# GATECH-EIC/PipeGCN

Hardware: AMD Instinct MI355X
Metric: epoch time (s), reddit 3-layer GraphSAGE (full-graph, pipelined) (lower is better)
Workload: dtype fp32; 1 GPU; model=graphsage-3L-h256, graph=reddit, num_nodes=232965, avg_degree=492, n_feat=602, n_class=41, pipeline=True, use_pp=False, norm=layer, parallelism=graph-partition dp1, num_halo=0, num_edges=114851422

## Files before the change

pipegcn_amd/csrc/bindings.cpp:

```cpp

#include "common.h"

static torch::Tensor spmm(torch::Tensor indptr, torch::Tensor indices,
                          torch::Tensor feat, torch::Tensor dst_scale,
                          torch::Tensor src_scale, torch::Tensor row_order,
                          int64_t num_rows) {
  if (feat.is_cuda()) {
    auto out = torch::empty({num_rows, feat.size(1)}, feat.options());
    spmm_csr_hip(indptr, indices, feat, dst_scale, src_scale, row_order,
                 out);
    return out;
  }
  if (feat.scalar_type() == torch::kBFloat16) {
    return spmm_cpu(indptr, indices, feat.to(torch::kFloat), dst_scale,
                    src_scale, num_rows)
        .to(torch::kBFloat16);
  }
  return spmm_cpu(indptr, indices, feat, dst_scale, src_scale, num_rows);
}

static torch::Tensor pack_rows(torch::Tensor x) {
  TORCH_CHECK(x.is_cuda() && x.dim() == 2, "pack_rows is the GPU path");
  auto packed = torch::empty({x.size(0), packed_layout(x.size(1)).stride_words},
                             x.options().dtype(torch::kInt));
  pack_rows_hip(x, packed);
  return packed;
}

static torch::Tensor spmm_packed(torch::Tensor indptr, torch::Tensor indices,
                                 torch::Tensor packed, int64_t F,
                                 torch::Tensor dst_scale,
                                 torch::Tensor row_order, int64_t num_rows) {
  TORCH_CHECK(packed.is_cuda(), "spmm_packed is the GPU path");
  auto out = torch::empty({num_rows, F},
                          packed.options().dtype(torch::kFloat));
  spmm_packed_hip(indptr, indices, packed, F, dst_scale, row_order, out);
  return out;
}

static torch::Tensor gather_rows(torch::Tensor src, torch::Tensor idx) {
  if (src.is_cuda()) {
    auto out = torch::empty({idx.numel(), src.size(1)}, src.options());
    gather_rows_hip(src, idx, out);
    return out;
  }
  return src.index_select(0, idx);
}

static void gather_rows_out(torch::Tensor src, torch::Tensor idx,
                            torch::Tensor out) {
  if (src.is_cuda()) {
    gather_rows_hip(src, idx, out);
  } else {
    torch::index_select_out(out, src, 0, idx);
  }
}

static void scatter_add_rows(torch::Tensor dst, torch::Tensor idx,
                             torch::Tensor src) {
  if (dst.is_cuda()) {
    scatter_add_rows_hip(dst, idx, src);
  } else {
    dst.index_add_(0, idx, src);
  }
}

static torch::Tensor sage_dual_gemm(torch::Tensor x1, torch::Tensor x2,
                                    torch::Tensor w1, torch::Tensor w2,
                                    torch::Tensor bias) {
  if (x1.is_cuda()) {
    auto out = torch::empty({x1.size(0), w1.size(0)}, x1.options());
// ... 23 lines not shown
  auto mask = torch::empty({(x.numel() + 7) / 8},
                           x.options().dtype(torch::kUInt8));
  dropout_fwd_hip(x, y, mask, p, seed);
  return {y, mask};
}

static torch::Tensor dropout_bwd(torch::Tensor dy, torch::Tensor mask,
                                 double p) {
  auto dx = torch::empty_like(dy);
  dropout_bwd_hip(dy.contiguous(), mask, dx, p);
  return dx;
}

static std::vector<torch::Tensor> layer_norm_relu_fwd(torch::Tensor x,
                                                      torch::Tensor w,
                                                      torch::Tensor b,
                                                      double eps, bool relu) {
  TORCH_CHECK(x.is_cuda(), "fused layer_norm_relu is the GPU path");
  auto y = torch::empty_like(x);
  auto xhat = torch::empty_like(x);
  auto rstd = torch::empty({x.size(0)}, x.options().dtype(torch::kFloat));
  layer_norm_relu_fwd_hip(x.contiguous(), w, b, eps, relu, y, xhat, rstd);
  return {y, xhat, rstd};
}

static std::vector<torch::Tensor> layer_norm_relu_bwd(
    torch::Tensor dy, torch::Tensor xhat, torch::Tensor rstd,
    torch::Tensor w, torch::Tensor b, bool relu) {
  auto dx = torch::empty_like(dy);
  const int64_t N = dy.size(0);
  const int64_t F = dy.size(1);
  const int64_t nblk = std::min<int64_t>(1024, (N + 3) / 4);
  auto dw_part = torch::empty({nblk * 4, F},
                              dy.options().dtype(torch::kFloat));
  auto db_part = torch::empty_like(dw_part);
  layer_norm_relu_bwd_hip(dy.contiguous(), xhat, rstd, w, b, relu, dx,
                          dw_part, db_part);
  return {dx, colsum_hip(dw_part), colsum_hip(db_part)};
}

static void ema_update(torch::Tensor avg, torch::Tensor x, double momentum) {
  if (avg.is_cuda()) {
    ema_update_hip(avg, x, momentum);
  } else {
    avg.mul_(momentum).add_(x, 1.0 - momentum);
  }
}

PYBIND11_MODULE(TORCH_EXTENSION_NAME, m) {
  m.doc() = "pipegcn_amd native core (gfx950 HIP kernels + host graph ops)";
  m.def("build_csr", &build_csr, "COO -> CSR (counting sort by dst)");
  m.def("partition_graph", &partition_graph_cpu,
        "BFS-grown + refined k-way partitioner (cut/vol objective)");
  m.def("spmm", &spmm, "CSR SpMM with fused scale epilogue (fwd & transpose)");
  m.def("pack_rows", &pack_rows,
        "fp32 [N, F] -> packed rows int32 [N, stride_words]");
  m.def("spmm_packed", &spmm_packed,
        "CSR SpMM over packed rows (fp32, dst_scale epilogue)");
  m.def("gather_rows", &gather_rows, "out[i,:] = src[idx[i],:]");
  m.def("gather_rows_out", &gather_rows_out,
        "gather into a preallocated out buffer");
  m.def("scatter_add_rows", &scatter_add_rows, "dst[idx[i],:] += src[i,:]");
  m.def("ema_update", &ema_update, "avg = m*avg + (1-m)*x");
  m.def("colsum", &colsum, "out[n] = sum_m x[m,n]");
  m.def("sage_dual_gemm", &sage_dual_gemm,
        "out = x1 @ w1^T + x2 @ w2^T + bias (MFMA fp32, fused)");
  m.def("dual_dgrad", &dual_dgrad_hip,
        "gx1 = g w1, gx2 = g w2 fused MFMA dgrad");
  m.def("dual_wgrad", &dual_wgrad_hip,
        "gw1 = g^T x1 [, gw2 = g^T x2] fused MFMA split-M wgrad");
  m.def("dropout_fwd", &dropout_fwd,
        "fused dropout, bitpacked mask -> (y, mask)");
  m.def("dropout_bwd", &dropout_bwd, "dx = mask ? dy/(1-p) : 0");
  m.def("layer_norm_relu_fwd", &layer_norm_relu_fwd,
        "fused LayerNorm[+ReLU] -> (y, xhat, rstd)");
  m.def("layer_norm_relu_bwd", &layer_norm_relu_bwd,
        "-> (dx, dweight, dbias)");
  m.def("gat_row_stats", &gat_row_stats_hip,
        "per-destination log-sum-exp of the GAT edge scores -> lse");
  m.def("gat_aggregate_fwd", &gat_aggregate_fwd_hip,
        "edge-softmax aggregation -> (out[, zc, csum])", py::arg("indptr"),
        py::arg("indices"), py::arg("z"), py::arg("el"), py::arg("er"),
        py::arg("lse"), py::arg("row_order"), py::arg("num_cols"),
        py::arg("num_heads"), py::arg("slope"), py::arg("with_aux"),
        py::arg("drop_key") = 0, py::arg("drop_thr") = 0,
        py::arg("drop_scale") = 1.0);
  m.def("gat_aggregate_bwd", &gat_aggregate_bwd_hip,
        "transpose edge-softmax aggregation over the CSC -> (dz, d_el)",
        py::arg("indptr"), py::arg("indices"), py::arg("g"), py::arg("z"),
        py::arg("el"), py::arg("er"), py::arg("lse"), py::arg("t"),
        py::arg("row_order"), py::arg("num_cols"), py::arg("num_heads"),
        py::arg("slope"), py::arg("drop_key") = 0, py::arg("drop_thr") = 0,
        py::arg("drop_scale") = 1.0);
  m.def("gat_dropout_keep", &gat_dropout_keep_hip,
        "attention-dropout keep bits of explicit (u, v) ids -> bool [n, H]",
        py::arg("u"), py::arg("v"), py::arg("num_heads"), py::arg("seed"),
        py::arg("p"));
  m.def("gatv2_fwd", &gatv2_fwd_hip,
        "GATv2 dynamic-attention aggregation over the CSR -> (out, lse)",
        py::arg("indptr"), py::arg("indices"), py::arg("zl"), py::arg("zr"),
        py::arg("attn"), py::arg("row_order"), py::arg("num_cols"),
        py::arg("num_heads"), py::arg("slope"), py::arg("drop_key") = 0,
        py::arg("drop_thr") = 0, py::arg("drop_scale") = 1.0);
  m.def("gatv2_bwd_dst", &gatv2_bwd_dst_hip,
        "GATv2 backward over the CSR -> (d_zr, pa)", py::arg("indptr"),
        py::arg("indices"), py::arg("g"), py::arg("zl"), py::arg("zr"),
        py::arg("attn"), py::arg("lse"), py::arg("t"), py::arg("row_order"),
// ... 13 lines not shown
```

pipegcn_amd/csrc/common.h:

```cpp
#pragma once

#include <torch/extension.h>

#include <cstdint>
#include <vector>


std::vector<torch::Tensor> build_csr(torch::Tensor u, torch::Tensor v,
                                     int64_t num_rows);

torch::Tensor partition_graph_cpu(torch::Tensor indptr, torch::Tensor indices,
                                  int64_t nparts, int64_t objective,
                                  double balance_slack, int64_t n_refine_passes,
                                  int64_t seed);

torch::Tensor spmm_cpu(torch::Tensor indptr, torch::Tensor indices,
                       torch::Tensor feat, torch::Tensor dst_scale,
                       torch::Tensor src_scale, int64_t num_rows);


void spmm_csr_hip(torch::Tensor indptr, torch::Tensor indices,
                  torch::Tensor feat, torch::Tensor dst_scale,
                  torch::Tensor src_scale, torch::Tensor row_order,
                  torch::Tensor out);

struct PackedLayout {
  int64_t mask_words;
  int64_t hdr_words;
  int64_t stride_words;
};
PackedLayout packed_layout(int64_t F);
void pack_rows_hip(torch::Tensor x, torch::Tensor packed);
void spmm_packed_hip(torch::Tensor indptr, torch::Tensor indices,
                     torch::Tensor packed, int64_t F, torch::Tensor dst_scale,
                     torch::Tensor row_order, torch::Tensor out);

void gather_rows_hip(torch::Tensor src, torch::Tensor idx, torch::Tensor out);

void scatter_add_rows_hip(torch::Tensor dst, torch::Tensor idx,
                          torch::Tensor src);

void ema_update_hip(torch::Tensor avg, torch::Tensor x, double momentum);

torch::Tensor colsum_hip(torch::Tensor x);

void dropout_fwd_hip(torch::Tensor x, torch::Tensor y, torch::Tensor mask,
                     double p, int64_t seed);
void dropout_bwd_hip(torch::Tensor dy, torch::Tensor mask, torch::Tensor dx,
                     double p);

void layer_norm_relu_fwd_hip(torch::Tensor x, torch::Tensor w,
                             torch::Tensor b, double eps, bool relu,
                             torch::Tensor y, torch::Tensor xhat,
                             torch::Tensor rstd);
std::vector<torch::Tensor> dual_dgrad_hip(torch::Tensor g, torch::Tensor w1,
                                          torch::Tensor w2);

std::vector<torch::Tensor> dual_wgrad_hip(torch::Tensor g, torch::Tensor x1,
                                          torch::Tensor x2);

void layer_norm_relu_bwd_hip(torch::Tensor dy, torch::Tensor xhat,
                             torch::Tensor rstd, torch::Tensor w,
                             torch::Tensor b, bool relu, torch::Tensor dx,
                             torch::Tensor dw_part, torch::Tensor db_part);

torch::Tensor gat_row_stats_hip(torch::Tensor indptr, torch::Tensor indices,
                                torch::Tensor el, torch::Tensor er,
                                int64_t num_cols, double slope);
std::vector<torch::Tensor> gat_aggregate_fwd_hip(
    torch::Tensor indptr, torch::Tensor indices, torch::Tensor z,
    torch::Tensor el, torch::Tensor er, torch::Tensor lse,
    torch::Tensor row_order, int64_t num_cols, int64_t H, double slope,
    bool with_aux, int64_t drop_key, int64_t drop_thr, double drop_scale);
std::vector<torch::Tensor> gat_aggregate_bwd_hip(
    torch::Tensor indptr, torch::Tensor indices, torch::Tensor g,
    torch::Tensor z, torch::Tensor el, torch::Tensor er, torch::Tensor lse,
    torch::Tensor t, torch::Tensor row_order, int64_t num_cols, int64_t H,
// ... 24 lines not shown
```

pipegcn_amd/csrc/hip/elementwise.hip:

```cpp

#include "../common.h"
#include "hip_util.h"

#include <hip/hip_bf16.h>
#include <hip/hip_runtime.h>

namespace {

__device__ inline void from_f32(float v, float* p) { *p = v; }
__device__ inline void from_f32(float v, __hip_bfloat16* p) {
  *p = __float2bfloat16(v);
}

__device__ inline float wave_sum(float v) {
#pragma unroll
  for (int off = 32; off > 0; off >>= 1) v += __shfl_xor(v, off, 64);
  return v;
}

__device__ inline uint64_t splitmix64(uint64_t z) {
  z += 0x9E3779B97F4A7C15ull;
  z = (z ^ (z >> 30)) * 0xBF58476D1CE4E5B9ull;
  z = (z ^ (z >> 27)) * 0x94D049BB133111EBull;
  return z ^ (z >> 31);
// ... 206 lines not shown
    float h[LN_MAXCH][LN_VEC];
    float s1 = 0.f, s2 = 0.f;
#pragma unroll
    for (int c = 0; c < LN_MAXCH; ++c) {
      if (c >= nch) break;
#pragma unroll
      for (int k = 0; k < LN_VEC; ++k) {
        const int f = (c * 64 + lane) * LN_VEC + k;
        float gg = 0.f, hh = 0.f;
        if (f < F) {
          hh = to_f32(hr[f]);
          gg = to_f32(dyr[f]);
          if (RELU && w[f] * hh + b[f] <= 0.f) gg = 0.f;
          acc_db[c][k] += gg;
          acc_dw[c][k] += gg * hh;
          gg *= w[f];
        }
        g[c][k] = gg;
        h[c][k] = hh;
        s1 += gg;
        s2 += gg * hh;
      }
    }
    s1 = wave_sum(s1) / F;
    s2 = wave_sum(s2) / F;
    T* dxr = dx + row * F;
#pragma unroll
    for (int c = 0; c < LN_MAXCH; ++c) {
      if (c >= nch) break;
#pragma unroll
      for (int k = 0; k < LN_VEC; ++k) {
        const int f = (c * 64 + lane) * LN_VEC + k;
        if (f >= F) break;
        from_f32(rs * (g[c][k] - s1 - h[c][k] * s2), &dxr[f]);
      }
    }
  }

  float* dwp = dw_part + wid * F;
  float* dbp = db_part + wid * F;
#pragma unroll
  for (int c = 0; c < LN_MAXCH; ++c) {
    if (c >= nch) break;
#pragma unroll
    for (int k = 0; k < LN_VEC; ++k) {
      const int f = (c * 64 + lane) * LN_VEC + k;
      if (f >= F) break;
      dwp[f] = acc_dw[c][k];
      dbp[f] = acc_db[c][k];
    }
  }
}

}

void dropout_fwd_hip(torch::Tensor x, torch::Tensor y, torch::Tensor mask,
                     double p, int64_t seed) {
  TORCH_CHECK(x.is_cuda() && x.is_contiguous() && y.is_contiguous());
  TORCH_CHECK(mask.scalar_type() == torch::kUInt8 && mask.is_contiguous());
  const int64_t n = x.numel();
  TORCH_CHECK(mask.numel() >= (n + 7) / 8);
  TORCH_CHECK(p >= 0.0 && p < 1.0);
  const uint32_t p16 = static_cast<uint32_t>(p * 65536.0 + 0.5);
  const float scale = 1.f / (1.f - p16 / 65536.f);
  const int64_t groups = (n + 7) / 8;
  const int threads = 256;
  const int64_t blocks =
      std::min<int64_t>((groups + threads - 1) / threads, 65535 * 8);
  const bool bf16 = x.scalar_type() == torch::kBFloat16;
  TORCH_CHECK(bf16 || x.scalar_type() == torch::kFloat);
  if (bf16)
    hipLaunchKernelGGL(HIP_KERNEL_NAME(dropout_fwd_kernel<__hip_bfloat16>),
                       dim3(blocks), dim3(threads), 0, current_stream(),
                       reinterpret_cast<__hip_bfloat16*>(x.data_ptr()),
                       reinterpret_cast<__hip_bfloat16*>(y.data_ptr()),
                       mask.data_ptr<uint8_t>(), (uint64_t)seed, p16, scale,
                       n);
  else
    hipLaunchKernelGGL(HIP_KERNEL_NAME(dropout_fwd_kernel<float>),
                       dim3(blocks), dim3(threads), 0, current_stream(),
                       x.data_ptr<float>(), y.data_ptr<float>(),
                       mask.data_ptr<uint8_t>(), (uint64_t)seed, p16, scale,
                       n);
  check_launch();
}

void dropout_bwd_hip(torch::Tensor dy, torch::Tensor mask, torch::Tensor dx,
                     double p) {
  TORCH_CHECK(dy.is_cuda() && dy.is_contiguous() && dx.is_contiguous());
  const int64_t n = dy.numel();
  const uint32_t p16 = static_cast<uint32_t>(p * 65536.0 + 0.5);
  const float scale = 1.f / (1.f - p16 / 65536.f);
  const int64_t groups = (n + 7) / 8;
  const int threads = 256;
  const int64_t blocks =
      std::min<int64_t>((groups + threads - 1) / threads, 65535 * 8);
  const bool bf16 = dy.scalar_type() == torch::kBFloat16;
  if (bf16)
    hipLaunchKernelGGL(HIP_KERNEL_NAME(dropout_bwd_kernel<__hip_bfloat16>),
                       dim3(blocks), dim3(threads), 0, current_stream(),
                       reinterpret_cast<__hip_bfloat16*>(dy.data_ptr()),
                       mask.data_ptr<uint8_t>(),
                       reinterpret_cast<__hip_bfloat16*>(dx.data_ptr()),
                       scale, n);
  else
    hipLaunchKernelGGL(HIP_KERNEL_NAME(dropout_bwd_kernel<float>),
// ... 80 lines not shown
```

pipegcn_amd/csrc/hip/kernels.hip:

```cpp

#include "../common.h"
#include "hip_util.h"

#include <hip/hip_bf16.h>
#include <hip/hip_runtime.h>

#include <cstdlib>
#include <vector>

namespace {

__device__ __forceinline__ void st_nt(float* p, float v) {
  __builtin_nontemporal_store(v, p);
}
__device__ __forceinline__ void st_nt(__hip_bfloat16* p, float v) {
  union {
    __hip_bfloat16 b;
    unsigned short u;
  } cv;
  cv.b = __float2bfloat16(v);
  __builtin_nontemporal_store(cv.u, reinterpret_cast<unsigned short*>(p));
}
__device__ __forceinline__ void st(float* p, float v) { *p = v; }
__device__ __forceinline__ void st(__hip_bfloat16* p, float v) {
  *p = __float2bfloat16(v);
}


template <typename T, int VEC, bool HAS_SRC_SCALE>
__global__ void spmm_csr_kernel(const int64_t* __restrict__ indptr,
                                const int32_t* __restrict__ indices,
                                const T* __restrict__ feat,
                                const float* __restrict__ dst_scale,
                                const float* __restrict__ src_scale,
                                const int32_t* __restrict__ row_order,
                                T* __restrict__ out, int64_t num_rows,
                                int64_t F, int64_t nchunks) {
  const int wave_in_block =
      __builtin_amdgcn_readfirstlane(static_cast<int>(threadIdx.x) / kWave);
  const int64_t waves_per_block = blockDim.x / kWave;
  const int64_t wave_global =
      static_cast<int64_t>(blockIdx.x) * waves_per_block + wave_in_block;
  const int lane = threadIdx.x & (kWave - 1);
  const int64_t nwaves = static_cast<int64_t>(gridDim.x) * waves_per_block;
  const int64_t npairs = num_rows * nchunks;

  for (int64_t pair = wave_global; pair < npairs; pair += nwaves) {
    int64_t r = pair / nchunks;
    const int64_t chunk = pair % nchunks;
    if (row_order) r = row_order[r];
    const int64_t f0 = chunk * (kWave * VEC) + lane * VEC;
    if (f0 >= F) continue;
    const bool full = (f0 + VEC <= F);

    float acc[VEC];
#pragma unroll
    for (int k = 0; k < VEC; ++k) acc[k] = 0.f;

    const int64_t e_begin = indptr[r];
    const int64_t e_end = indptr[r + 1];
    int64_t e = e_begin;

    if (full) {
      for (; e < e_end && (e & 3); ++e) {
        const int64_t u = indices[e];
        const float s = HAS_SRC_SCALE ? src_scale[u] : 1.f;
#pragma unroll
        for (int k = 0; k < VEC; ++k)
          acc[k] += s * to_f32(feat[u * F + f0 + k]);
      }
      for (; e + 4 <= e_end; e += 4) {
        const int32x4 uu = *reinterpret_cast<const int32x4*>(indices + e);
        const int64_t u0 = uu[0];
        const int64_t u1 = uu[1];
        const int64_t u2 = uu[2];
        const int64_t u3 = uu[3];
        float s0 = 1.f, s1 = 1.f, s2 = 1.f, s3 = 1.f;
        if (HAS_SRC_SCALE) {
          s0 = src_scale[u0];
          s1 = src_scale[u1];
          s2 = src_scale[u2];
          s3 = src_scale[u3];
        }
        float v0[VEC], v1[VEC], v2[VEC], v3[VEC];
#pragma unroll
        for (int k = 0; k < VEC; ++k) v0[k] = to_f32(feat[u0 * F + f0 + k]);
#pragma unroll
        for (int k = 0; k < VEC; ++k) v1[k] = to_f32(feat[u1 * F + f0 + k]);
#pragma unroll
        for (int k = 0; k < VEC; ++k) v2[k] = to_f32(feat[u2 * F + f0 + k]);
#pragma unroll
        for (int k = 0; k < VEC; ++k) v3[k] = to_f32(feat[u3 * F + f0 + k]);
        if (HAS_SRC_SCALE) {
#pragma unroll
          for (int k = 0; k < VEC; ++k)
            acc[k] += s0 * v0[k] + s1 * v1[k] + s2 * v2[k] + s3 * v3[k];
        } else {
#pragma unroll
          for (int k = 0; k < VEC; ++k)
            acc[k] += v0[k] + v1[k] + v2[k] + v3[k];
        }
      }
      for (; e < e_end; ++e) {
        const int64_t u = indices[e];
        const float s = HAS_SRC_SCALE ? src_scale[u] : 1.f;
#pragma unroll
        for (int k = 0; k < VEC; ++k)
          acc[k] += s * to_f32(feat[u * F + f0 + k]);
      }
      const float s = dst_scale ? dst_scale[r] : 1.f;
#pragma unroll
      for (int k = 0; k < VEC; ++k) st_nt(out + r * F + f0 + k, acc[k] * s);
    } else {
      for (; e < e_end; ++e) {
        const int64_t u = indices[e];
        const float s = HAS_SRC_SCALE ? src_scale[u] : 1.f;
        for (int k = 0; k < VEC && f0 + k < F; ++k)
          acc[k] += s * to_f32(feat[u * F + f0 + k]);
      }
      const float s = dst_scale ? dst_scale[r] : 1.f;
      for (int k = 0; k < VEC && f0 + k < F; ++k)
        st(out + r * F + f0 + k, acc[k] * s);
    }
  }
}

template <typename T, int VEC>
void launch_spmm(const int64_t* indptr, const int32_t* indices,
                 const T* feat, const float* dst_scale,
                 const float* src_scale, const int32_t* row_order, T* out,
                 int64_t num_rows, int64_t F, hipStream_t stream) {
  const int64_t nchunks = (F + kWave * VEC - 1) / (kWave * VEC);
  constexpr int threads = 256;
  static_assert(threads % kWave == 0);
  const int64_t blocks = grid_for(num_rows * nchunks, threads);
  auto launch = [&](auto kern) {
    hipLaunchKernelGGL(kern, dim3(blocks), dim3(threads), 0, stream, indptr,
                       indices, feat, dst_scale, src_scale, row_order, out,
                       num_rows, F, nchunks);
  };
  if (src_scale)
    launch(HIP_KERNEL_NAME(spmm_csr_kernel<T, VEC, true>));
  else
    launch(HIP_KERNEL_NAME(spmm_csr_kernel<T, VEC, false>));
  check_launch();
}


template <typename T, int VEC, bool SCATTER_ADD>
__global__ void rowcopy_kernel(const T* __restrict__ src,
                               const int64_t* __restrict__ idx,
                               T* __restrict__ dst, int64_t nrows,
                               int64_t F, int64_t nchunks) {
  const int64_t wave_global =
      (static_cast<int64_t>(blockIdx.x) * blockDim.x + threadIdx.x) / kWave;
  const int lane = threadIdx.x & (kWave - 1);
  const int64_t nwaves =
      (static_cast<int64_t>(gridDim.x) * blockDim.x) / kWave;
  const int64_t npairs = nrows * nchunks;
  for (int64_t pair = wave_global; pair < npairs; pair += nwaves) {
    const int64_t i = pair / nchunks;
    const int64_t f0 = pair % nchunks * (kWave * VEC) + lane * VEC;
    if (f0 >= F) continue;
    const int64_t j = idx[i];
    if (f0 + VEC <= F) {
#pragma unroll
      for (int k = 0; k < VEC; ++k) {
        if (SCATTER_ADD)
          st(dst + j * F + f0 + k, to_f32(dst[j * F + f0 + k]) +
                                       to_f32(src[i * F + f0 + k]));
        else
          dst[i * F + f0 + k] = src[j * F + f0 + k];
      }
    } else {
      for (int k = 0; f0 + k < F; ++k) {
        if (SCATTER_ADD)
          st(dst + j * F + f0 + k, to_f32(dst[j * F + f0 + k]) +
                                       to_f32(src[i * F + f0 + k]));
        else
          dst[i * F + f0 + k] = src[j * F + f0 + k];
      }
    }
  }
}

template <typename T, int VEC, bool SCATTER_ADD>
void launch_rowcopy(const T* src, const int64_t* idx, T* dst,
                    int64_t nrows, int64_t F, hipStream_t stream) {
  const int64_t nchunks = (F + kWave * VEC - 1) / (kWave * VEC);
  const int threads = 256;
  const int64_t blocks = grid_for(nrows * nchunks, threads);
  hipLaunchKernelGGL(HIP_KERNEL_NAME(rowcopy_kernel<T, VEC, SCATTER_ADD>),
                     dim3(blocks), dim3(threads), 0, stream, src, idx, dst,
                     nrows, F, nchunks);
  check_launch();
}

// ... 18 lines not shown

template <int VEC>
__global__ void colsum_partial_kernel(const float* __restrict__ x,
                                      float* __restrict__ partials,
                                      int64_t M, int64_t F,
                                      int64_t rows_per_blk) {
  const int64_t blk = blockIdx.x;
  const int64_t r0 = blk * rows_per_blk;
  const int64_t r1 = min(r0 + rows_per_blk, M);
  for (int64_t f0 = static_cast<int64_t>(threadIdx.x) * VEC; f0 < F;
       f0 += 256 * VEC) {
    float acc[VEC];
#pragma unroll
    for (int k = 0; k < VEC; ++k) acc[k] = 0.f;
    if (f0 + VEC <= F) {
      for (int64_t r = r0; r < r1; ++r) {
#pragma unroll
        for (int k = 0; k < VEC; ++k) acc[k] += x[r * F + f0 + k];
      }
#pragma unroll
      for (int k = 0; k < VEC; ++k) partials[blk * F + f0 + k] = acc[k];
    } else {
      for (int64_t r = r0; r < r1; ++r)
        for (int k = 0; f0 + k < F; ++k) acc[k] += x[r * F + f0 + k];
      for (int k = 0; f0 + k < F; ++k) partials[blk * F + f0 + k] = acc[k];
    }
  }
}

int pick_vec(int64_t F, int64_t num_rows, int64_t elem_size = 4) {
  if (const char* e = std::getenv("PIPEGCN_SPMM_VEC")) {
    int v = std::atoi(e);
    if ((v == 8 || v == 4 || v == 2 || v == 1) && F % v == 0 &&
        v * elem_size <= 16)
      return v;
  }
  const bool big = num_rows >= (1 << 20);
  const std::initializer_list<int> pref =
      big ? std::initializer_list<int>{16, 8, 4}
          : std::initializer_list<int>{8, 16, 4};
  for (int bytes : pref) {
    if (bytes < elem_size) continue;
    const int v = bytes / static_cast<int>(elem_size);
    if (F % v == 0) return v;
  }
  return 1;
}

}

template <typename T>
void spmm_dispatch(torch::Tensor& indptr, torch::Tensor& indices,
                   torch::Tensor& feat, const float* dsp, const float* ssp,
                   const int32_t* rop, torch::Tensor& out, int64_t num_rows,
                   int64_t F, int vec, hipStream_t stream) {
  const T* fp = reinterpret_cast<const T*>(feat.data_ptr());
  T* op = reinterpret_cast<T*>(out.data_ptr());
  const int64_t* ip = indptr.data_ptr<int64_t>();
  const int32_t* xp = indices.data_ptr<int32_t>();
  dispatch_vec(vec, [&](auto v) {
    launch_spmm<T, v.value>(ip, xp, fp, dsp, ssp, rop, op, num_rows, F,
                            stream);
  });
}

void spmm_csr_hip(torch::Tensor indptr, torch::Tensor indices,
                  torch::Tensor feat, torch::Tensor dst_scale,
                  torch::Tensor src_scale, torch::Tensor row_order,
                  torch::Tensor out) {
  TORCH_CHECK(feat.is_cuda() && out.is_cuda(), "spmm_csr_hip: device tensors");
  const bool bf16 = feat.scalar_type() == torch::kBFloat16;
  TORCH_CHECK(bf16 || feat.scalar_type() == torch::kFloat,
              "spmm: fp32 or bf16 only");
  TORCH_CHECK(out.scalar_type() == feat.scalar_type());
  TORCH_CHECK(feat.is_contiguous() && out.is_contiguous());
  TORCH_CHECK(indptr.scalar_type() == torch::kLong &&
              indices.scalar_type() == torch::kInt);
  const int64_t num_rows = out.size(0);
  const int64_t num_src = feat.size(0);
  const int64_t F = feat.size(1);
  TORCH_CHECK(out.size(1) == F && indptr.numel() == num_rows + 1);
  const float* dsp = nullptr;
  if (dst_scale.defined() && dst_scale.numel() > 0) {
    TORCH_CHECK(dst_scale.is_contiguous() && dst_scale.numel() == num_rows);
    TORCH_CHECK(dst_scale.scalar_type() == torch::kFloat);
    dsp = dst_scale.data_ptr<float>();
  }
  const float* ssp = nullptr;
  if (src_scale.defined() && src_scale.numel() > 0) {
    TORCH_CHECK(src_scale.is_contiguous() && src_scale.numel() == num_src);
    TORCH_CHECK(src_scale.scalar_type() == torch::kFloat);
    ssp = src_scale.data_ptr<float>();
  }
  const int32_t* rop = nullptr;
  if (row_order.defined() && row_order.numel() > 0) {
    TORCH_CHECK(row_order.is_contiguous() && row_order.numel() == num_rows &&
                row_order.scalar_type() == torch::kInt);
    rop = row_order.data_ptr<int32_t>();
  }
  auto stream = current_stream();
  const int vec = pick_vec(F, num_rows, bf16 ? 2 : 4);
  if (bf16)
    spmm_dispatch<__hip_bfloat16>(indptr, indices, feat, dsp, ssp, rop, out,
                                  num_rows, F, vec, stream);
  else
    spmm_dispatch<float>(indptr, indices, feat, dsp, ssp, rop, out, num_rows,
                         F, vec, stream);
}

template <typename T, bool SCATTER_ADD>
void rowcopy_dispatch(torch::Tensor& src, torch::Tensor& idx,
                      torch::Tensor& dst, int64_t n, int64_t F,
                      int vec, hipStream_t stream) {
  const T* sp = reinterpret_cast<const T*>(src.data_ptr());
  T* dp = reinterpret_cast<T*>(dst.data_ptr());
  const int64_t* ixp = idx.data_ptr<int64_t>();
  dispatch_vec(vec, [&](auto v) {
    launch_rowcopy<T, v.value, SCATTER_ADD>(sp, ixp, dp, n, F, stream);
  });
}

void gather_rows_hip(torch::Tensor src, torch::Tensor idx, torch::Tensor out) {
  TORCH_CHECK(src.is_cuda() && idx.is_cuda() && out.is_cuda());
  const bool bf16 = src.scalar_type() == torch::kBFloat16;
  TORCH_CHECK(bf16 || src.scalar_type() == torch::kFloat);
  TORCH_CHECK(out.scalar_type() == src.scalar_type() &&
              idx.scalar_type() == torch::kLong);
  TORCH_CHECK(src.is_contiguous() && out.is_contiguous());
  const int64_t F = src.size(1);
  const int64_t n = idx.numel();
  TORCH_CHECK(out.size(0) == n && out.size(1) == F);
  auto stream = current_stream();
  const int vec = pick_vec(F, 0, bf16 ? 2 : 4);
  if (bf16)
    rowcopy_dispatch<__hip_bfloat16, false>(src, idx, out, n, F, vec, stream);
  else
    rowcopy_dispatch<float, false>(src, idx, out, n, F, vec, stream);
}

void scatter_add_rows_hip(torch::Tensor dst, torch::Tensor idx,
                          torch::Tensor src) {
  TORCH_CHECK(dst.is_cuda() && idx.is_cuda() && src.is_cuda());
  const bool bf16 = dst.scalar_type() == torch::kBFloat16;
  TORCH_CHECK(bf16 || dst.scalar_type() == torch::kFloat);
  TORCH_CHECK(src.scalar_type() == dst.scalar_type() &&
              idx.scalar_type() == torch::kLong);
  TORCH_CHECK(src.is_contiguous() && dst.is_contiguous());
  const int64_t F = dst.size(1);
  const int64_t n = idx.numel();
  TORCH_CHECK(src.size(0) == n && src.size(1) == F);
  auto stream = current_stream();
  const int vec = pick_vec(F, 0, bf16 ? 2 : 4);
  if (bf16)
    rowcopy_dispatch<__hip_bfloat16, true>(src, idx, dst, n, F, vec, stream);
  else
    rowcopy_dispatch<float, true>(src, idx, dst, n, F, vec, stream);
}

torch::Tensor colsum_hip(torch::Tensor x) {
  TORCH_CHECK(x.is_cuda() && x.dim() == 2 && x.is_contiguous());
// ... 31 lines not shown
```

pipegcn_amd/ops/__init__.py:

```python
from __future__ import annotations

import math
import os
from typing import Optional

import torch

from pipegcn_amd import native
from pipegcn_amd.graph.csr import CSR, HaloGraph


def _row_order(matrix: CSR) -> torch.Tensor:
    return matrix.row_order if matrix.row_order is not None else torch.Tensor()


def _tune_row_order(csr: CSR, feat, s, ss) -> bool:
    import time

    nat = torch.Tensor()
    times = {}
    for key, ro in (("lpt", csr.row_order), ("nat", nat)):
        native().spmm(csr.indptr, csr.indices, feat, s, ss, ro,
                      csr.num_rows)
        torch.cuda.synchronize()
        t0 = time.perf_counter()
        for _ in range(2):
            native().spmm(csr.indptr, csr.indices, feat, s, ss, ro,
                          csr.num_rows)
        torch.cuda.synchronize()
        times[key] = time.perf_counter() - t0
    return times["lpt"] <= times["nat"]


def spmm(csr: CSR, feat: torch.Tensor,
         scale: Optional[torch.Tensor] = None,
         src_scale: Optional[torch.Tensor] = None) -> torch.Tensor:
    if feat.shape[0] < csr.num_cols:
        raise ValueError(
            f"spmm: feat has {feat.shape[0]} rows but the graph references "
            f"{csr.num_cols} source nodes (an under-sized feat would be an "
            "out-of-bounds GPU gather)")
    s = scale if scale is not None else torch.Tensor()
    ss = src_scale if src_scale is not None else torch.Tensor()
    feat = feat.contiguous()
    ro = _row_order(csr)
    if (feat.is_cuda and csr.row_order is not None
            and csr.nnz * feat.shape[1] >= (1 << 30)
            and os.environ.get("PIPEGCN_SPMM_AUTOTUNE", "1") == "1"):
        cache = getattr(csr, "_lpt_choice", None)
        if cache is None:
            cache = {}
            csr._lpt_choice = cache
        use_lpt = cache.get(feat.shape[1])
        if use_lpt is None:
            free, _ = torch.cuda.mem_get_info(feat.device)
            out_bytes = csr.num_rows * feat.shape[1] * feat.element_size()
            if free < 3 * out_bytes + (2 << 30):
                use_lpt = True
            else:
                use_lpt = _tune_row_order(csr, feat, s, ss)
            cache[feat.shape[1]] = use_lpt
        if not use_lpt:
            ro = torch.Tensor()
    return native().spmm(csr.indptr, csr.indices, feat, s, ss,
                         ro, csr.num_rows)


def packed_row_layout(F: int):
    mask_words = (F + 31) // 32
    hdr_words = (2 * mask_words + 3) // 4 * 4
    stride_words = (hdr_words + F + 8 + 31) // 32 * 32
    return mask_words, hdr_words, stride_words


def pack_rows_reference(x: torch.Tensor) -> torch.Tensor:
    if x.dim() != 2 or x.dtype != torch.float32:
        raise ValueError("pack_rows_reference: fp32 [N, F] only")
    N, F = x.shape
    W, hdr, stride = packed_row_layout(F)
    nz = x != 0
    nzp = torch.zeros(N, W * 32, dtype=torch.int64, device=x.device)
    nzp[:, :F] = nz
    nzp = nzp.view(N, W, 32)
    mask = (nzp << torch.arange(32, device=x.device)).sum(-1)
    cnt = nzp.sum(-1)
    prefix = cnt.cumsum(-1) - cnt
    out = torch.zeros(N, stride, dtype=torch.int32, device=x.device)
    out[:, 0:2 * W:2] = ((mask + 2 ** 31) % 2 ** 32 - 2 ** 31).int()
    out[:, 1:2 * W:2] = prefix.int()
    rank = nz.long().cumsum(-1) - 1
    rows = torch.arange(N, device=x.device).unsqueeze(1).expand(N, F)
    out[rows[nz], hdr + rank[nz]] = x.contiguous().view(torch.int32)[nz]
    return out


def unpack_rows_reference(packed: torch.Tensor, F: int) -> torch.Tensor:
    W, hdr, stride = packed_row_layout(F)
    if packed.dim() != 2 or packed.shape[1] != stride \
            or packed.dtype != torch.int32:
        raise ValueError("unpack_rows_reference: not packed rows of width "
                         f"{F}")
    N = packed.shape[0]
    mask = packed[:, 0:2 * W:2].long() & _M32
    prefix = packed[:, 1:2 * W:2].long()
    bits = (mask.unsqueeze(-1) >> torch.arange(32, device=packed.device)) & 1
    rank = prefix.unsqueeze(-1) + bits.cumsum(-1) - bits
    nz = bits.view(N, W * 32)[:, :F].bool()
    rank = rank.view(N, W * 32)[:, :F]
    vals = packed[:, hdr:].gather(1, rank.clamp(max=stride - hdr - 1))
    return torch.where(nz, vals, torch.zeros_like(vals)).view(torch.float32)


def pack_rows(x: torch.Tensor) -> torch.Tensor:
    if x.is_cuda:
        return native().pack_rows(x.contiguous())
    return pack_rows_reference(x)


def _spmm_packed_width(F: int) -> bool:
    return F >= 64


def _spmm_packed_route(feat: torch.Tensor) -> bool:
    if (not feat.is_cuda or feat.dtype != torch.float32
            or os.environ.get("PIPEGCN_SPMM_PACKED", "1") == "0"
            or not _spmm_packed_width(feat.shape[1])):
        return False
    free, _ = torch.cuda.mem_get_info(feat.device)
    need = feat.shape[0] * packed_row_layout(feat.shape[1])[2] * 4
    return free >= need + (2 << 30)


def spmm_packed(csr: CSR, feat: torch.Tensor,
                scale: Optional[torch.Tensor] = None) -> torch.Tensor:
    if feat.shape[0] < csr.num_cols:
        raise ValueError(
            f"spmm_packed: feat has {feat.shape[0]} rows but the graph "
            f"references {csr.num_cols} source nodes (an under-sized feat "
            "would be an out-of-bounds GPU gather)")
    if not feat.is_cuda or feat.dtype != torch.float32 or feat.dim() != 2:
        raise ValueError("spmm_packed: fp32 [N, F] GPU tensors only")
    s = scale if scale is not None else torch.Tensor()
    ro = _row_order(csr)
    if getattr(csr, "_lpt_choice", {}).get(feat.shape[1]) is False:
        ro = torch.Tensor()
    packed = native().pack_rows(feat.contiguous())
    return native().spmm_packed(csr.indptr, csr.indices, packed,
                                feat.shape[1], s, ro, csr.num_rows)


class _SpmmMean(torch.autograd.Function):

    @staticmethod
    def forward(ctx, graph: HaloGraph, feat: torch.Tensor,
                inv_deg: torch.Tensor):
        ctx.graph = graph
        ctx.save_for_backward(inv_deg)
        if _spmm_packed_route(feat):
            return spmm_packed(graph.csr, feat, inv_deg)
        return spmm(graph.csr, feat, inv_deg)

    @staticmethod
    def backward(ctx, grad_out: torch.Tensor):
        (inv_deg,) = ctx.saved_tensors
        g = ctx.graph
        if g.csc.nnz > grad_out.numel():
            grad_feat = spmm(
                g.csc,
                grad_out * inv_deg.unsqueeze(1).to(grad_out.dtype), None)
        else:
            grad_feat = spmm(g.csc, grad_out.contiguous(), None,
                             src_scale=inv_deg)
        return None, grad_feat, None


def spmm_mean(graph: HaloGraph, feat: torch.Tensor,
              inv_deg: torch.Tensor) -> torch.Tensor:
    return _SpmmMean.apply(graph, feat, inv_deg)


def _gat_check(csr: CSR, z, el, er, num_heads: int) -> None:
    if num_heads < 1 or z.dim() != 2 or z.shape[1] % num_heads != 0:
        raise ValueError(
            f"gat_aggregate: feature width {tuple(z.shape)} is not "
            f"num_heads*D for num_heads={num_heads}")
    if el.dim() != 2 or er.dim() != 2 or el.shape[1] != num_heads \
            or er.shape[1] != num_heads:
        raise ValueError(
            f"gat_aggregate: el/er must be [nodes, {num_heads}], got "
            f"{tuple(el.shape)} and {tuple(er.shape)}")
    if z.shape[0] < csr.num_cols or el.shape[0] < csr.num_cols:
        raise ValueError(
            f"gat_aggregate: z/el have {z.shape[0]}/{el.shape[0]} rows but "
            f"the graph references {csr.num_cols} source nodes (an "
            "under-sized tensor would be an out-of-bounds GPU gather)")
    if er.shape[0] != csr.num_rows:
        raise ValueError(
            f"gat_aggregate: er has {er.shape[0]} rows, the graph has "
            f"{csr.num_rows} destination nodes")


_M32 = 0xFFFFFFFF
_M64 = 0xFFFFFFFFFFFFFFFF


def _gat_dropout_params(seed: int, p: float):
    x = (int(seed) + 0x9E3779B97F4A7C15) & _M64
    x = ((x ^ (x >> 30)) * 0xBF58476D1CE4E5B9) & _M64
    x = ((x ^ (x >> 27)) * 0x94D049BB133111EB) & _M64
    x ^= x >> 31
    thr = min(int(math.floor(p * 4294967296.0 + 0.5)), _M32)
    return x & _M32, thr, 1.0 / (1.0 - p)


def _gat_keep_hash(u: torch.Tensor, v: torch.Tensor, num_heads: int,
                   key: int) -> torch.Tensor:
    u = u.long() & _M32
    v = v.long() & _M32
    h = torch.arange(num_heads, dtype=torch.int64, device=u.device)
    x = ((u * 0x9E3779B1 + v * 0x85EBCA77).unsqueeze(-1)
         + h * 0xC2B2AE3D + key) & _M32
    x = x ^ (x >> 16)
# ... 400 lines not shown
```

Before: 0.08175 s/epoch.

## Redirect SpMM backward gathers of trailing all-zero gradient rows to one row

Adds a fused kernel that scales the backward gradient rows by inverse degree and also records 1 + the index of the last row with any non-zero value. The transpose SpMM then clamps every source index to that bound, so reads of trailing all-zero rows hit one shared zero row that stays in cache instead of fetching distinct rows. The aim is to cut gather traffic in the mean-aggregation backward, which applies when non-training nodes with zero loss gradient sit at the end of the node order. It also replaces the separate elementwise multiply with the fused scale kernel, at the cost of an extra atomic and a memset per call.

```diff
diff --git a/pipegcn_amd/csrc/bindings.cpp b/pipegcn_amd/csrc/bindings.cpp
--- a/pipegcn_amd/csrc/bindings.cpp
+++ b/pipegcn_amd/csrc/bindings.cpp
@@ -1,14 +1,17 @@
 
 #include "common.h"
+
+#include <optional>
 
 static torch::Tensor spmm(torch::Tensor indptr, torch::Tensor indices,
                           torch::Tensor feat, torch::Tensor dst_scale,
                           torch::Tensor src_scale, torch::Tensor row_order,
-                          int64_t num_rows) {
+                          int64_t num_rows,
+                          std::optional<torch::Tensor> n_live) {
   if (feat.is_cuda()) {
     auto out = torch::empty({num_rows, feat.size(1)}, feat.options());
     spmm_csr_hip(indptr, indices, feat, dst_scale, src_scale, row_order,
-                 out);
+                 out, n_live.value_or(torch::Tensor()));
     return out;
   }
   if (feat.scalar_type() == torch::kBFloat16) {
@@ -17,6 +20,17 @@
         .to(torch::kBFloat16);
   }
   return spmm_cpu(indptr, indices, feat, dst_scale, src_scale, num_rows);
+}
+
+static std::vector<torch::Tensor> scale_rows_live(torch::Tensor g,
+                                                  torch::Tensor inv) {
+  TORCH_CHECK(g.is_cuda() && g.dim() == 2,
+              "scale_rows_live is the GPU path");
+  if (g.size(0) > 1 && g.size(1) > 1 && g.stride(1) != 1) g = g.contiguous();
+  auto scaled = torch::empty({g.size(0), g.size(1)}, g.options());
+  auto n_live = torch::empty({1}, g.options().dtype(torch::kInt));
+  scale_rows_live_hip(g, inv, scaled, n_live);
+  return {scaled, n_live};
 }
 
 static torch::Tensor pack_rows(torch::Tensor x) {
@@ -146,7 +160,12 @@
   m.def("build_csr", &build_csr, "COO -> CSR (counting sort by dst)");
   m.def("partition_graph", &partition_graph_cpu,
         "BFS-grown + refined k-way partitioner (cut/vol objective)");
-  m.def("spmm", &spmm, "CSR SpMM with fused scale epilogue (fwd & transpose)");
+  m.def("spmm", &spmm, "CSR SpMM with fused scale epilogue (fwd & transpose)",
+        py::arg("indptr"), py::arg("indices"), py::arg("feat"),
+        py::arg("dst_scale"), py::arg("src_scale"), py::arg("row_order"),
+        py::arg("num_rows"), py::arg("n_live") = py::none());
+  m.def("scale_rows_live", &scale_rows_live,
+        "g * inv per row -> (scaled, n_live = 1 + last non-zero row, int32)");
   m.def("pack_rows", &pack_rows,
         "fp32 [N, F] -> packed rows int32 [N, stride_words]");
   m.def("spmm_packed", &spmm_packed,
diff --git a/pipegcn_amd/csrc/common.h b/pipegcn_amd/csrc/common.h
--- a/pipegcn_amd/csrc/common.h
+++ b/pipegcn_amd/csrc/common.h
@@ -22,7 +22,10 @@
 void spmm_csr_hip(torch::Tensor indptr, torch::Tensor indices,
                   torch::Tensor feat, torch::Tensor dst_scale,
                   torch::Tensor src_scale, torch::Tensor row_order,
-                  torch::Tensor out);
+                  torch::Tensor out, torch::Tensor n_live = {});
+
+void scale_rows_live_hip(torch::Tensor g, torch::Tensor inv,
+                         torch::Tensor scaled, torch::Tensor n_live);
 
 struct PackedLayout {
   int64_t mask_words;
diff --git a/pipegcn_amd/csrc/hip/elementwise.hip b/pipegcn_amd/csrc/hip/elementwise.hip
--- a/pipegcn_amd/csrc/hip/elementwise.hip
+++ b/pipegcn_amd/csrc/hip/elementwise.hip
@@ -282,6 +282,161 @@
   }
 }
 
+
+template <typename T>
+struct RowScaleElem;
+template <>
+struct RowScaleElem<float> {
+  using raw = float;
+  static __device__ __forceinline__ float scale(float inv) { return inv; }
+  static __device__ __forceinline__ float mul(float v, float s) {
+    return v * s;
+  }
+  static __device__ __forceinline__ bool nonzero(float v) { return v != 0.f; }
+};
+template <>
+struct RowScaleElem<__hip_bfloat16> {
+  using raw = unsigned short;
+  static __device__ __forceinline__ unsigned short round(float f) {
+    const uint32_t b = __float_as_uint(f);
+    if (f != f) return 0x7FC0;
+    return static_cast<unsigned short>((b + 0x7FFFu + ((b >> 16) & 1u)) >> 16);
+  }
+  static __device__ __forceinline__ float widen(unsigned short h) {
+    return __uint_as_float(static_cast<uint32_t>(h) << 16);
+  }
+  static __device__ __forceinline__ float scale(float inv) {
+    return widen(round(inv));
+  }
+  static __device__ __forceinline__ unsigned short mul(unsigned short v,
+                                                       float s) {
+    return round(widen(v) * s);
+  }
+  static __device__ __forceinline__ bool nonzero(unsigned short v) {
+    return (v & 0x7FFFu) != 0;
+  }
+};
+
+template <typename R, int VEC>
+struct alignas(sizeof(R) * VEC) RowScalePack {
+  R v[VEC];
+};
+
+constexpr int kScaleInFlight = 4;
+
+template <typename T, int VEC>
+__global__ void scale_rows_live_kernel(const T* __restrict__ g,
+                                       const float* __restrict__ inv,
+                                       T* __restrict__ scaled,
+                                       int32_t* __restrict__ n_live,
+                                       int64_t N, int64_t F,
+                                       int64_t g_stride, int64_t nchunks) {
+  using E = RowScaleElem<T>;
+  using Pack = RowScalePack<typename E::raw, VEC>;
+  __shared__ int blk_live;
+  if (threadIdx.x == 0) blk_live = 0;
+  __syncthreads();
+
+  const int wave_in_block =
+      __builtin_amdgcn_readfirstlane(static_cast<int>(threadIdx.x) / kWave);
+  const int64_t waves_per_block = blockDim.x / kWave;
+  const int64_t wave_global =
+      static_cast<int64_t>(blockIdx.x) * waves_per_block + wave_in_block;
+  const int lane = threadIdx.x & (kWave - 1);
+  const int64_t nwaves = static_cast<int64_t>(gridDim.x) * waves_per_block;
+  const int64_t npairs = N * nchunks;
+  const auto* gp = reinterpret_cast<const typename E::raw*>(g);
+  auto* sp = reinterpret_cast<typename E::raw*>(scaled);
+
+  int live = 0;
+  for (int64_t p0 = wave_global; p0 < npairs;
+       p0 += kScaleInFlight * nwaves) {
+    Pack p[kScaleInFlight];
+    float s[kScaleInFlight];
+    int64_t row[kScaleInFlight], f0[kScaleInFlight];
+    bool on[kScaleInFlight];
+#pragma unroll
+    for (int j = 0; j < kScaleInFlight; ++j) {
+      const int64_t pair = p0 + j * nwaves;
+      const int64_t pc = min(pair, npairs - 1);
+      row[j] = pc / nchunks;
+      f0[j] = pc % nchunks * (kWave * VEC) + lane * VEC;
+      on[j] = pair < npairs && f0[j] < F;
+      p[j] = *reinterpret_cast<const Pack*>(gp + row[j] * g_stride +
+                                            min(f0[j], F - VEC));
+      s[j] = E::scale(inv[row[j]]);
+    }
+#pragma unroll
+    for (int j = 0; j < kScaleInFlight; ++j) {
+      if (!on[j]) continue;
+      bool nz = false;
+#pragma unroll
+      for (int k = 0; k < VEC; ++k) {
+        p[j].v[k] = E::mul(p[j].v[k], s[j]);
+        nz |= E::nonzero(p[j].v[k]);
+      }
+      *reinterpret_cast<Pack*>(sp + row[j] * F + f0[j]) = p[j];
+      if (nz) live = max(live, static_cast<int>(row[j]) + 1);
+    }
+  }
+  if (live > 0) atomicMax(&blk_live, live);
+  __syncthreads();
+  if (threadIdx.x == 0 && blk_live > 0) atomicMax(n_live, blk_live);
+}
+
+}
+
+void scale_rows_live_hip(torch::Tensor g, torch::Tensor inv,
+                         torch::Tensor scaled, torch::Tensor n_live) {
+  TORCH_CHECK(g.is_cuda() && g.dim() == 2 && scaled.is_cuda() &&
+              inv.is_cuda() && n_live.is_cuda());
+  const bool bf16 = g.scalar_type() == torch::kBFloat16;
+  TORCH_CHECK(bf16 || g.scalar_type() == torch::kFloat,
+              "scale_rows_live: fp32 or bf16 only");
+  const int64_t N = g.size(0);
+  const int64_t F = g.size(1);
+  TORCH_CHECK(N < (int64_t{1} << 31) - 1, "scale_rows_live: int32 row count");
+  TORCH_CHECK(N <= 1 || F <= 1 || g.stride(1) == 1,
+              "scale_rows_live: unit column stride");
+  TORCH_CHECK(scaled.scalar_type() == g.scalar_type() &&
+              scaled.is_contiguous() && scaled.size(0) == N &&
+              scaled.size(1) == F);
+  TORCH_CHECK(inv.scalar_type() == torch::kFloat && inv.is_contiguous() &&
+              inv.numel() == N);
+  TORCH_CHECK(n_live.scalar_type() == torch::kInt && n_live.numel() == 1);
+  auto stream = current_stream();
+  HIP_CHECK(hipMemsetAsync(n_live.data_ptr(), 0, sizeof(int32_t), stream));
+  if (N == 0 || F == 0) return;
+  const int64_t g_stride = N > 1 ? g.stride(0) : F;
+  const int64_t elem = bf16 ? 2 : 4;
+  int vec = static_cast<int>(16 / elem);
+  while (vec > 1 &&
+         (F % vec || g_stride % vec || !aligned_to(g.data_ptr(), vec * elem) ||
+          !aligned_to(scaled.data_ptr(), vec * elem)))
+    vec >>= 1;
+  constexpr int threads = 256;
+  const int64_t nchunks = (F + kWave * vec - 1) / (kWave * vec);
+  const int64_t blocks = std::min<int64_t>(
+      (N * nchunks + threads / kWave * kScaleInFlight - 1) /
+          (threads / kWave * kScaleInFlight),
+      2048);
+  auto launch = [&](auto tptr, auto kern) {
+    using TP = decltype(tptr);
+    hipLaunchKernelGGL(kern, dim3(blocks), dim3(threads), 0, stream,
+                       reinterpret_cast<const TP>(g.data_ptr()),
+                       inv.data_ptr<float>(),
+                       reinterpret_cast<TP>(scaled.data_ptr()),
+                       n_live.data_ptr<int32_t>(), N, F, g_stride, nchunks);
+  };
+  dispatch_vec(vec, [&](auto v) {
+    if (bf16)
+      launch((__hip_bfloat16*)nullptr,
+             HIP_KERNEL_NAME(scale_rows_live_kernel<__hip_bfloat16, v.value>));
+    else if constexpr (v.value <= 4)
+      launch((float*)nullptr,
+             HIP_KERNEL_NAME(scale_rows_live_kernel<float, v.value>));
+  });
+  check_launch();
 }
 
 void dropout_fwd_hip(torch::Tensor x, torch::Tensor y, torch::Tensor mask,
diff --git a/pipegcn_amd/csrc/hip/kernels.hip b/pipegcn_amd/csrc/hip/kernels.hip
--- a/pipegcn_amd/csrc/hip/kernels.hip
+++ b/pipegcn_amd/csrc/hip/kernels.hip
@@ -27,7 +27,7 @@
 }
 
 
-template <typename T, int VEC, bool HAS_SRC_SCALE>
+template <typename T, int VEC, bool HAS_SRC_SCALE, bool HAS_LIVE>
 __global__ void spmm_csr_kernel(const int64_t* __restrict__ indptr,
                                 const int32_t* __restrict__ indices,
                                 const T* __restrict__ feat,
@@ -35,7 +35,15 @@
                                 const float* __restrict__ src_scale,
                                 const int32_t* __restrict__ row_order,
                                 T* __restrict__ out, int64_t num_rows,
-                                int64_t F, int64_t nchunks) {
+                                int64_t F, int64_t nchunks,
+                                const int32_t* __restrict__ n_live) {
+  static_assert(!(HAS_SRC_SCALE && HAS_LIVE),
+                "the redirect would also redirect the scale's index");
+  int32_t live = 0;
+  if constexpr (HAS_LIVE) live = max(*n_live, 0);
+  auto node = [&](int32_t u) -> int64_t {
+    return HAS_LIVE ? min(u, live) : u;
+  };
   const int wave_in_block =
       __builtin_amdgcn_readfirstlane(static_cast<int>(threadIdx.x) / kWave);
   const int64_t waves_per_block = blockDim.x / kWave;
@@ -63,7 +71,7 @@
 
     if (full) {
       for (; e < e_end && (e & 3); ++e) {
-        const int64_t u = indices[e];
+        const int64_t u = node(indices[e]);
         const float s = HAS_SRC_SCALE ? src_scale[u] : 1.f;
 #pragma unroll
         for (int k = 0; k < VEC; ++k)
@@ -71,10 +79,10 @@
       }
       for (; e + 4 <= e_end; e += 4) {
         const int32x4 uu = *reinterpret_cast<const int32x4*>(indices + e);
-        const int64_t u0 = uu[0];
-        const int64_t u1 = uu[1];
-        const int64_t u2 = uu[2];
-        const int64_t u3 = uu[3];
+        const int64_t u0 = node(uu[0]);
+        const int64_t u1 = node(uu[1]);
+        const int64_t u2 = node(uu[2]);
+        const int64_t u3 = node(uu[3]);
         float s0 = 1.f, s1 = 1.f, s2 = 1.f, s3 = 1.f;
         if (HAS_SRC_SCALE) {
           s0 = src_scale[u0];
@@ -102,7 +110,7 @@
         }
       }
       for (; e < e_end; ++e) {
-        const int64_t u = indices[e];
+        const int64_t u = node(indices[e]);
         const float s = HAS_SRC_SCALE ? src_scale[u] : 1.f;
 #pragma unroll
         for (int k = 0; k < VEC; ++k)
@@ -113,7 +121,7 @@
       for (int k = 0; k < VEC; ++k) st_nt(out + r * F + f0 + k, acc[k] * s);
     } else {
       for (; e < e_end; ++e) {
-        const int64_t u = indices[e];
+        const int64_t u = node(indices[e]);
         const float s = HAS_SRC_SCALE ? src_scale[u] : 1.f;
         for (int k = 0; k < VEC && f0 + k < F; ++k)
           acc[k] += s * to_f32(feat[u * F + f0 + k]);
@@ -128,8 +136,9 @@
 template <typename T, int VEC>
 void launch_spmm(const int64_t* indptr, const int32_t* indices,
                  const T* feat, const float* dst_scale,
-                 const float* src_scale, const int32_t* row_order, T* out,
-                 int64_t num_rows, int64_t F, hipStream_t stream) {
+                 const float* src_scale, const int32_t* row_order,
+                 const int32_t* n_live, T* out, int64_t num_rows, int64_t F,
+                 hipStream_t stream) {
   const int64_t nchunks = (F + kWave * VEC - 1) / (kWave * VEC);
   constexpr int threads = 256;
   static_assert(threads % kWave == 0);
@@ -137,12 +146,14 @@
   auto launch = [&](auto kern) {
     hipLaunchKernelGGL(kern, dim3(blocks), dim3(threads), 0, stream, indptr,
                        indices, feat, dst_scale, src_scale, row_order, out,
-                       num_rows, F, nchunks);
+                       num_rows, F, nchunks, n_live);
   };
-  if (src_scale)
-    launch(HIP_KERNEL_NAME(spmm_csr_kernel<T, VEC, true>));
+  if (n_live)
+    launch(HIP_KERNEL_NAME(spmm_csr_kernel<T, VEC, false, true>));
+  else if (src_scale)
+    launch(HIP_KERNEL_NAME(spmm_csr_kernel<T, VEC, true, false>));
   else
-    launch(HIP_KERNEL_NAME(spmm_csr_kernel<T, VEC, false>));
+    launch(HIP_KERNEL_NAME(spmm_csr_kernel<T, VEC, false, false>));
   check_launch();
 }
 
@@ -267,14 +278,14 @@
 template <typename T>
 void spmm_dispatch(torch::Tensor& indptr, torch::Tensor& indices,
                    torch::Tensor& feat, const float* dsp, const float* ssp,
-                   const int32_t* rop, torch::Tensor& out, int64_t num_rows,
-                   int64_t F, int vec, hipStream_t stream) {
+                   const int32_t* rop, const int32_t* nlp, torch::Tensor& out,
+                   int64_t num_rows, int64_t F, int vec, hipStream_t stream) {
   const T* fp = reinterpret_cast<const T*>(feat.data_ptr());
   T* op = reinterpret_cast<T*>(out.data_ptr());
   const int64_t* ip = indptr.data_ptr<int64_t>();
   const int32_t* xp = indices.data_ptr<int32_t>();
   dispatch_vec(vec, [&](auto v) {
-    launch_spmm<T, v.value>(ip, xp, fp, dsp, ssp, rop, op, num_rows, F,
+    launch_spmm<T, v.value>(ip, xp, fp, dsp, ssp, rop, nlp, op, num_rows, F,
                             stream);
   });
 }
@@ -282,7 +293,7 @@
 void spmm_csr_hip(torch::Tensor indptr, torch::Tensor indices,
                   torch::Tensor feat, torch::Tensor dst_scale,
                   torch::Tensor src_scale, torch::Tensor row_order,
-                  torch::Tensor out) {
+                  torch::Tensor out, torch::Tensor n_live) {
   TORCH_CHECK(feat.is_cuda() && out.is_cuda(), "spmm_csr_hip: device tensors");
   const bool bf16 = feat.scalar_type() == torch::kBFloat16;
   TORCH_CHECK(bf16 || feat.scalar_type() == torch::kFloat,
@@ -313,14 +324,24 @@
                 row_order.scalar_type() == torch::kInt);
     rop = row_order.data_ptr<int32_t>();
   }
+  const int32_t* nlp = nullptr;
+  if (n_live.defined() && n_live.numel() > 0) {
+    TORCH_CHECK(n_live.is_cuda() && n_live.numel() == 1 &&
+                    n_live.scalar_type() == torch::kInt,
+                "spmm: n_live is one int32 in device memory");
+    TORCH_CHECK(ssp == nullptr,
+                "spmm: n_live and src_scale do not combine (the redirect "
+                "would pick another row's scale)");
+    nlp = n_live.data_ptr<int32_t>();
+  }
   auto stream = current_stream();
   const int vec = pick_vec(F, num_rows, bf16 ? 2 : 4);
   if (bf16)
-    spmm_dispatch<__hip_bfloat16>(indptr, indices, feat, dsp, ssp, rop, out,
-                                  num_rows, F, vec, stream);
+    spmm_dispatch<__hip_bfloat16>(indptr, indices, feat, dsp, ssp, rop, nlp,
+                                  out, num_rows, F, vec, stream);
   else
-    spmm_dispatch<float>(indptr, indices, feat, dsp, ssp, rop, out, num_rows,
-                         F, vec, stream);
+    spmm_dispatch<float>(indptr, indices, feat, dsp, ssp, rop, nlp, out,
+                         num_rows, F, vec, stream);
 }
 
 template <typename T, bool SCATTER_ADD>
diff --git a/pipegcn_amd/ops/__init__.py b/pipegcn_amd/ops/__init__.py
--- a/pipegcn_amd/ops/__init__.py
+++ b/pipegcn_amd/ops/__init__.py
@@ -34,7 +34,8 @@
 
 def spmm(csr: CSR, feat: torch.Tensor,
          scale: Optional[torch.Tensor] = None,
-         src_scale: Optional[torch.Tensor] = None) -> torch.Tensor:
+         src_scale: Optional[torch.Tensor] = None,
+         n_live: Optional[torch.Tensor] = None) -> torch.Tensor:
     if feat.shape[0] < csr.num_cols:
         raise ValueError(
             f"spmm: feat has {feat.shape[0]} rows but the graph references "
@@ -62,8 +63,15 @@
             cache[feat.shape[1]] = use_lpt
         if not use_lpt:
             ro = torch.Tensor()
+    if n_live is None:
+        return native().spmm(csr.indptr, csr.indices, feat, s, ss,
+                             ro, csr.num_rows)
     return native().spmm(csr.indptr, csr.indices, feat, s, ss,
-                         ro, csr.num_rows)
+                         ro, csr.num_rows, n_live)
+
+
+def scale_rows_live(g: torch.Tensor, inv: torch.Tensor):
+    return native().scale_rows_live(g, inv)
 
 
 def packed_row_layout(F: int):
@@ -165,9 +173,15 @@
         (inv_deg,) = ctx.saved_tensors
         g = ctx.graph
         if g.csc.nnz > grad_out.numel():
-            grad_feat = spmm(
-                g.csc,
-                grad_out * inv_deg.unsqueeze(1).to(grad_out.dtype), None)
+            if grad_out.is_cuda:
+                scaled, n_live = scale_rows_live(grad_out, inv_deg)
+                if os.environ.get("PIPEGCN_SPMM_LIVE", "1") == "0":
+                    n_live = None
+                grad_feat = spmm(g.csc, scaled, None, n_live=n_live)
+            else:
+                grad_feat = spmm(
+                    g.csc,
+                    grad_out * inv_deg.unsqueeze(1).to(grad_out.dtype), None)
         else:
             grad_feat = spmm(g.csc, grad_out.contiguous(), None,
                              src_scale=inv_deg)
```

Measured after the change: 0.07664 s/epoch, median of 6. -6.2%, faster.
